# Clemapfel/kmer_index

Measured on NVIDIA B200. Metric: search_queries_per_s, higher is better.
Workload: dtype u32

## Files before the change

kmer_index_b200/csrc/build_kernels.cu:

```cuda
#include "radix.cuh"
#include "launch.h"

namespace kb {

__global__ void __launch_bounds__(256) pack_text_kernel(const uint8_t *__restrict__ ranks, uint64_t n, uint32_t bits,
                                                        uint32_t sigma, uint64_t n_words, uint64_t *__restrict__ words,
                                                        uint32_t *__restrict__ error_flag) {
    const uint64_t w = (uint64_t)blockIdx.x * blockDim.x + threadIdx.x;
    if (w >= n_words) return;
    const uint32_t spw = 64 / bits;
    const uint64_t s0 = w * spw;
    uint64_t word = 0;
    bool bad = false;
    if (s0 + spw <= n && ((uintptr_t)(ranks + s0) & 7) == 0) {
        const uint64_t *src = reinterpret_cast<const uint64_t *>(ranks + s0);
        for (uint32_t j = 0; j < spw; j += 8) {
            const uint64_t v = src[j >> 3];
#pragma unroll
            for (uint32_t b = 0; b < 8; ++b) {
                const uint32_t r = (uint32_t)(v >> (8 * b)) & 0xFF;
                bad |= r >= sigma;
                word |= (uint64_t)r << (64 - bits * (j + b + 1));
            }
        }
// ... 475 lines not shown
    const int tid = threadIdx.x;
    const uint64_t tile_begin = (uint64_t)blockIdx.x * kTile;
    const uint64_t tile_end = min(tile_begin + kTile, n_kmers + 1);
    const uint32_t nb = (uint32_t)(tile_end - tile_begin);
    const bool edge = tile_begin == 0 || tile_end == n_kmers + 1;

    const uint64_t i0 = tile_begin + (uint64_t)tid * ITEMS;
    const KeyT k_base = tile_begin ? keys[tile_begin - 1] : (KeyT)0;
    KeyT k[ITEMS + 1];
    k[0] = (i0 >= 1 && i0 - 1 < n_kmers) ? keys[i0 - 1] : (KeyT)0;
    if (i0 + ITEMS <= n_kmers) {
        constexpr int kPerVec = 16 / (int)sizeof(KeyT);
        const uint4 *p = reinterpret_cast<const uint4 *>(keys + i0);
#pragma unroll
        for (int v = 0; v < ITEMS / kPerVec; ++v) {
            const uint4 q = p[v];
            if (sizeof(KeyT) == 4) {
                k[1 + 4 * v] = (KeyT)q.x;
                k[2 + 4 * v] = (KeyT)q.y;
                k[3 + 4 * v] = (KeyT)q.z;
                k[4 + 4 * v] = (KeyT)q.w;
            } else {
                k[1 + 2 * v] = (KeyT)(((uint64_t)q.y << 32) | q.x);
                k[2 + 2 * v] = (KeyT)(((uint64_t)q.w << 32) | q.z);
            }
        }
    } else {
#pragma unroll
        for (int j = 0; j < ITEMS; ++j) k[j + 1] = (i0 + j < n_kmers) ? keys[i0 + j] : (KeyT)0;
    }
#pragma unroll
    for (int t = 0; t < kSlab / (kDirThreads * 4); ++t)
        *reinterpret_cast<uint4 *>(slab + (t * kDirThreads + tid) * 4) = make_uint4(0, 0, 0, 0);

    const uint32_t b0 = (uint32_t)tid * ITEMS;
    if (!edge) {
        const uint32_t slot_base = (uint32_t)(k_base >> shift);
        uint32_t rel[ITEMS + 1];
#pragma unroll
        for (int j = 0; j <= ITEMS; ++j) rel[j] = (uint32_t)(k[j] >> shift) - slot_base;
        uint32_t head[ITEMS];
#pragma unroll
        for (int j = 0; j < ITEMS; ++j) head[j] = rel[j + 1] > rel[j] ? rel[j] : 0xFFFFFFFFu;
        if (tid == kDirThreads - 1) s_end = rel[ITEMS];
        __syncthreads();
        directory_rounds<uint32_t, ITEMS>(slab, warp_last, head, (uint32_t)i0, (uint32_t)s_end,
                                          dir + ((uint64_t)slot_base + 1));
    } else {
        const uint64_t base = tile_begin ? (uint64_t)(k_base >> shift) + 1 : 0;
        uint64_t head[ITEMS];
#pragma unroll
        for (int j = 0; j < ITEMS; ++j) {
            const uint64_t i = i0 + j;
            head[j] = ~0ull;
            if (b0 + j < nb) {
                const uint64_t lo = (i == 0) ? 0 : (uint64_t)(k[j] >> shift) + 1;
                const uint64_t hi = (i == n_kmers) ? dir_entries : (uint64_t)(k[j + 1] >> shift) + 1;
                if (hi > lo) head[j] = lo - base;
                if (b0 + j == nb - 1) s_end = hi - base;
            }
        }
        __syncthreads();
        directory_rounds<uint64_t, ITEMS>(slab, warp_last, head, (uint32_t)i0, s_end, dir + base);
    }
}

template <typename KeyT, int ITEMS>
static void launch_directory_fill_t(const KeyT *d_keys, uint64_t n_kmers, uint32_t shift, uint64_t dir_entries, uint32_t *d_dir,
                                    cudaStream_t stream) {
    const uint64_t tile = (uint64_t)kDirThreads * ITEMS;
    const uint64_t blocks = (n_kmers + 1 + tile - 1) / tile;
    cudaFuncSetAttribute(directory_fill_kernel<KeyT, ITEMS>, cudaFuncAttributePreferredSharedMemoryCarveout, 100);
    directory_fill_kernel<KeyT, ITEMS><<<(unsigned)blocks, kDirThreads, 0, stream>>>(d_keys, n_kmers, shift, dir_entries, d_dir);
}

void launch_directory_fill(const void *d_keys, uint32_t key_bytes, uint64_t n_kmers, uint32_t shift, uint64_t dir_entries,
                           uint32_t *d_dir, cudaStream_t stream) {
    if (key_bytes == 8)
        launch_directory_fill_t<uint64_t, 8>((const uint64_t *)d_keys, n_kmers, shift, dir_entries, d_dir, stream);
    else
        launch_directory_fill_t<uint32_t, 8>((const uint32_t *)d_keys, n_kmers, shift, dir_entries, d_dir, stream);
}

template <typename Source, int BITS, bool BYTE>
static void launch_scatter_bits(const Source &src, uint64_t n, uint32_t shift, uint32_t mask, const uint32_t *d_tile_base,
                                typename Source::key_type *d_out_keys, uint32_t *d_out_vals, cudaStream_t stream) {
    using Smem = ScatterSmem<typename Source::key_type, (Source::kAtomicItems != 0)>;
    const uint32_t n_tiles = (uint32_t)((n + kSortTile - 1) / kSortTile);
    cudaFuncSetAttribute(radix_scatter_kernel<Source, BITS, BYTE>, cudaFuncAttributeMaxDynamicSharedMemorySize, (int)sizeof(Smem));
    radix_scatter_kernel<Source, BITS, BYTE>
        <<<n_tiles, kSortThreads, sizeof(Smem), stream>>>(src, n, shift, mask, d_tile_base, d_out_keys, d_out_vals);
}

template <typename Source>
static void launch_scatter(const Source &src, uint64_t n, uint32_t shift, uint32_t mask, const uint32_t *d_tile_base,
                           typename Source::key_type *d_out_keys, uint32_t *d_out_vals, cudaStream_t stream) {
    const int bits = __builtin_popcount(mask);
    if (bits <= 5)
        launch_scatter_bits<Source, 5, false>(src, n, shift, mask, d_tile_base, d_out_keys, d_out_vals, stream);
    else if (bits == 6)
        launch_scatter_bits<Source, 6, false>(src, n, shift, mask, d_tile_base, d_out_keys, d_out_vals, stream);
    else if (bits == 7)
        launch_scatter_bits<Source, 7, false>(src, n, shift, mask, d_tile_base, d_out_keys, d_out_vals, stream);
    else if (sizeof(typename Source::key_type) == 4 && (shift & 7) == 0) {
        if constexpr (sizeof(typename Source::key_type) == 4)
            launch_scatter_bits<Source, 8, true>(src, n, shift, mask, d_tile_base, d_out_keys, d_out_vals, stream);
    } else
        launch_scatter_bits<Source, 8, false>(src, n, shift, mask, d_tile_base, d_out_keys, d_out_vals, stream);
}

void launch_column_scan(uint32_t *d_tile_hist, uint32_t n_tiles, uint32_t *d_chunk_sums, cudaStream_t stream) {
    const uint32_t n_chunks = (n_tiles + kScanChunk - 1) / kScanChunk;
    column_sum_kernel<<<n_chunks, kRadix, 0, stream>>>(d_tile_hist, n_tiles, d_chunk_sums);
    column_base_kernel<<<1, kRadix * kBaseSlices, 0, stream>>>(d_chunk_sums, n_chunks);
    column_apply_kernel<<<n_chunks, kRadix, 0, stream>>>(d_tile_hist, n_tiles, d_chunk_sums);
}

void launch_hist_text(const PackedText &text, uint32_t k, uint64_t n_kmers, uint32_t shift, uint32_t mask,
                      uint32_t *d_tile_hist, cudaStream_t stream) {
    const uint32_t n_tiles = (uint32_t)((n_kmers + kSortTile - 1) / kSortTile);
    if (k * text.bits > 64) {
        radix_hist_kernel<<<n_tiles, kSortThreads, 0, stream>>>(WideTextSource{text, k}, n_kmers, shift, mask, d_tile_hist);
        return;
    }
    radix_hist_text_kernel<<<n_tiles, kSortThreads, 0, stream>>>(text, k, n_kmers, shift, mask, d_tile_hist);
}

void launch_hist_pairs(const void *d_keys, uint32_t key_bytes, uint64_t n, uint32_t shift, uint32_t mask,
                       uint32_t *d_tile_hist, cudaStream_t stream) {
    const uint32_t n_tiles = (uint32_t)((n + kSortTile - 1) / kSortTile);
    if (key_bytes == 8) {
        PairSource<uint64_t> src{(const uint64_t *)d_keys, nullptr};
        radix_hist_kernel<<<n_tiles, kSortThreads, 0, stream>>>(src, n, shift, mask, d_tile_hist);
    } else {
        radix_hist_keys32_kernel<<<n_tiles, kSortThreads, 0, stream>>>((const uint32_t *)d_keys, n, shift, mask, d_tile_hist);
    }
}

void launch_scatter_text(const PackedText &text, uint32_t k, uint32_t key_bytes, uint64_t n_kmers, uint32_t shift,
                         uint32_t mask, const uint32_t *d_tile_base, void *d_out_keys, uint32_t *d_out_vals,
                         cudaStream_t stream) {
    if (k * text.bits > 64)
        launch_scatter(WideTextSource{text, k}, n_kmers, shift, mask, d_tile_base, (uint64_t *)d_out_keys, d_out_vals, stream);
    else if (key_bytes == 8)
        launch_scatter(TextSource<uint64_t>{text, k}, n_kmers, shift, mask, d_tile_base, (uint64_t *)d_out_keys, d_out_vals, stream);
    else
        launch_scatter(TextSource<uint32_t>{text, k}, n_kmers, shift, mask, d_tile_base, (uint32_t *)d_out_keys, d_out_vals, stream);
}

void launch_scatter_pairs(const void *d_keys, const uint32_t *d_vals, uint32_t key_bytes, uint64_t n, uint32_t shift,
                          uint32_t mask, const uint32_t *d_tile_base, void *d_out_keys, uint32_t *d_out_vals,
                          cudaStream_t stream) {
    if (key_bytes == 8)
        launch_scatter(PairSource<uint64_t>{(const uint64_t *)d_keys, d_vals}, n, shift, mask, d_tile_base,
                       (uint64_t *)d_out_keys, d_out_vals, stream);
    else
        launch_scatter(PairSource<uint32_t>{(const uint32_t *)d_keys, d_vals}, n, shift, mask, d_tile_base,
                       (uint32_t *)d_out_keys, d_out_vals, stream);
}

uint32_t sort_tile_size() { return kSortTile; }
uint32_t scan_chunk_tiles() { return kScanChunk; }

}
```

kmer_index_b200/csrc/capi.cu:

```cuda
#include <algorithm>
#include <atomic>
#include <condition_variable>
#include <chrono>
#include <cmath>
#include <cstdio>
#include <cstdlib>
#include <cstring>
#include <mutex>
#include <unordered_map>
#include <new>
#include <string>
#include <system_error>
#include <thread>
#include <vector>

#include "host_pack.h"
#include "launch.h"
#include "radix.cuh"

namespace {

thread_local std::string g_last_error;

int fail(int code, const std::string &msg) {
// ... 340 lines not shown
    return p;
}

void pinned_put(void *p, size_t cap) {
    if (!p) return;
    {
        std::lock_guard<std::mutex> lock(g_pinned_mu);
        if (g_pinned_cache.size() < 32) {
            g_pinned_cache.emplace_back(p, cap);
            return;
        }
    }
    cudaFreeHost(p);
}

struct SchemeHost {
    std::vector<uint32_t> ks;
    std::vector<uint32_t> sum_off;
    std::vector<uint8_t> sum_elem, use_multi;
};

void build_scheme(SchemeHost *ix) {
    const uint32_t R = kb::kQuerySizeRange;
    std::vector<uint32_t> all_ks(ix->ks);
    std::sort(all_ks.begin(), all_ks.end(), [](uint32_t a, uint32_t b) { return a > b; });
    std::vector<uint32_t> high;
    for (uint32_t k : all_ks)
        if (k >= 9) high.push_back(k);
    std::vector<uint32_t> len(R, 0), last(R, 0), prev(R, 0);
    ix->use_multi.assign(R, 0);
    for (uint32_t k : high)
        if (k < R) {
            len[k] = 1;
            last[k] = k;
            ix->use_multi[k] = 1;
        }
    for (uint32_t q = all_ks.front() + 1; q < R; ++q)
        for (uint32_t k : high)
            if (len[q - k] != 0) {
                len[q] = len[q - k] + 1;
                last[q] = k;
                prev[q] = q - k;
                ix->use_multi[q] = 1;
                break;
            }
    for (uint32_t q = 0; q < R; ++q) {
        if (len[q] != 0) continue;
        uint32_t best = all_ks.front();
        if (q < all_ks.front()) {
            for (uint32_t k : all_ks)
                if (q <= k && k - q < best - q) best = k;
        } else {
            auto waste = [q](uint32_t k) { return ((q + k - 1) / k) * k - q; };
            for (uint32_t k : all_ks)
                if (waste(k) < waste(best)) best = k;
        }
        len[q] = 1;
        last[q] = best;
    }
    auto elem_of = [ix](uint32_t k) {
        for (size_t i = 0; i < ix->ks.size(); ++i)
            if (ix->ks[i] == k) return (uint8_t)i;
        return (uint8_t)0;
    };
    ix->sum_off.assign(R + 2, 0);
    uint64_t total = 0;
    for (uint32_t q = 0; q < R; ++q) {
        ix->sum_off[q] = (uint32_t)total;
        total += len[q];
    }
    ix->sum_off[R] = (uint32_t)total;
    ix->sum_off[R + 1] = (uint32_t)total;
    ix->sum_elem.assign(total, 0);
    for (uint32_t q = 0; q < R; ++q) {
        uint64_t o = (uint64_t)ix->sum_off[q] + len[q];
        uint32_t c = q;
        for (uint32_t j = 0; j < len[q]; ++j) {
            ix->sum_elem[--o] = elem_of(last[c]);
            c = prev[c];
        }
    }
}

int sort_element_tiled(kmer_b200_index *ix, uint32_t k, HostElement &he, uint32_t digit_bits, KeyRange part, uint64_t *n_sorted) {
    using namespace kb;
    cudaStream_t st = ix->stream;
    Profiler &pf = ix->prof;
    const uint64_t n_text_kmers = ix->n - k + 1;
    const uint32_t key_bytes = he.key_bytes;
    const bool partial = part.lo != 0 || part.hi != fast_pow(ix->sigma, (uint8_t)k);
    PackedText text{ix->d_text, ix->n, ix->bits, ix->sigma};
    uint64_t n_kmers = n_text_kmers;
    uint32_t sort_bits = he.key_bits;
    void *f_keys = nullptr;
    uint32_t *f_vals = nullptr;
    if (partial) {
        const uint32_t ft = filter_tiles(n_text_kmers);
        uint64_t *tile_counts = nullptr, *block_sums = nullptr;
        KB_TRY(dev_alloc(ix, &tile_counts, (uint64_t)ft + 1, false));
        KB_TRY(dev_alloc(ix, &block_sums, offsets_scan_blocks(ft) + 1, false));
        pf.begin(K_HIST_TEXT, (double)n_text_kmers * ix->bits / 8.0);
        launch_owned_count(text, k, n_text_kmers, part.lo, part.hi, tile_counts, st);
        pf.end();
        launch_offsets_scan(tile_counts, ft, block_sums, st);
        KB_CUDA(cudaMemcpyAsync(&ix->h_pinned[6], tile_counts + ft, sizeof(uint64_t), cudaMemcpyDeviceToHost, st));
        KB_CUDA(cudaStreamSynchronize(st));
        n_kmers = ix->h_pinned[6];
        KB_TRY(dev_alloc(ix, (uint8_t **)&f_keys, std::max<uint64_t>(n_kmers, 1) * key_bytes, true));
        KB_TRY(dev_alloc(ix, &f_vals, std::max<uint64_t>(n_kmers, 1), true));
        pf.begin(K_SCATTER_TEXT, (double)n_text_kmers * ix->bits / 8.0 + 8.0 * n_kmers);
        launch_owned_write(text, k, n_text_kmers, part.lo, part.hi, tile_counts, (uint32_t *)f_keys, f_vals, st);
        pf.end();
        dev_free(ix, tile_counts);
        dev_free(ix, block_sums);
        sort_bits = std::max<uint32_t>(1, bit_length(part.hi - part.lo - 1));
    }
    *n_sorted = n_kmers;
    he.sort_passes = (sort_bits + digit_bits - 1) / digit_bits;
    const uint32_t bits_per_pass = (sort_bits + he.sort_passes - 1) / he.sort_passes;
    const uint32_t mask = (1u << bits_per_pass) - 1;
    const uint32_t n_tiles = (uint32_t)((n_kmers + sort_tile_size() - 1) / sort_tile_size());
    const uint32_t n_chunks = (n_tiles + scan_chunk_tiles() - 1) / scan_chunk_tiles();
    const double text_bytes = (double)n_kmers * ix->bits / 8.0;
    const double hist_bytes = (double)n_tiles * kRadix * 4;
    void *keys[2] = {nullptr, nullptr};
    uint32_t *vals[2] = {nullptr, nullptr};
    uint32_t *tile_hist = nullptr, *chunk_sums = nullptr;
    auto alloc_keys = [&](void **p) { return dev_alloc(ix, (uint8_t **)p, std::max<uint64_t>(n_kmers, 1) * key_bytes, true); };
    KB_TRY(dev_alloc(ix, &tile_hist, (uint64_t)std::max(n_tiles, 1u) * kRadix, false));
    KB_TRY(dev_alloc(ix, &chunk_sums, (uint64_t)std::max(n_chunks, 1u) * kRadix, false));
    int cur = 0;
    uint32_t first_pair_pass = 1;
    if (partial) {
        keys[0] = f_keys;
        vals[0] = f_vals;
        first_pair_pass = 0;
    } else {
        KB_TRY(alloc_keys(&keys[0]));
        KB_TRY(dev_alloc(ix, &vals[0], n_kmers, true));
        pf.begin(K_HIST_TEXT, text_bytes + hist_bytes);
        launch_hist_text(text, k, n_kmers, 0, mask, tile_hist, st);
        pf.end();
        pf.begin(K_COLUMN_SCAN, 3 * hist_bytes, 3);
        launch_column_scan(tile_hist, n_tiles, chunk_sums, st);
        pf.end();
        pf.begin(K_SCATTER_TEXT, text_bytes + hist_bytes + (4.0 + key_bytes) * n_kmers);
        launch_scatter_text(text, k, key_bytes, n_kmers, 0, mask, tile_hist, keys[0], vals[0], st);
        pf.end();
    }
    for (uint32_t p = first_pair_pass; p < he.sort_passes && n_kmers > 0; ++p) {
        const int nxt = cur ^ 1;
        if (!keys[nxt]) {
            KB_TRY(alloc_keys(&keys[nxt]));
            KB_TRY(dev_alloc(ix, &vals[nxt], n_kmers, true));
        }
        const uint32_t shift = p * bits_per_pass;
        pf.begin(K_HIST_PAIRS, (double)key_bytes * n_kmers + hist_bytes);
        launch_hist_pairs(keys[cur], key_bytes, n_kmers, shift, mask, tile_hist, st);
        pf.end();
        pf.begin(K_COLUMN_SCAN, 3 * hist_bytes, 3);
        launch_column_scan(tile_hist, n_tiles, chunk_sums, st);
        pf.end();
        pf.begin(K_SCATTER_PAIRS, 2.0 * (4.0 + key_bytes) * n_kmers + hist_bytes);
        launch_scatter_pairs(keys[cur], vals[cur], key_bytes, n_kmers, shift, mask, tile_hist, keys[nxt], vals[nxt], st);
        pf.end();
        cur = nxt;
    }
    KB_CUDA(cudaGetLastError());
    if (keys[cur ^ 1]) {
        dev_free(ix, (uint8_t *)keys[cur ^ 1]);
        dev_free(ix, vals[cur ^ 1]);
        ix->device_bytes -= std::max<uint64_t>(n_kmers, 1) * (sizeof(uint32_t) + key_bytes);
    }
    dev_free(ix, tile_hist);
    dev_free(ix, chunk_sums);
    he.d_keys = keys[cur];
    he.d_pos = vals[cur];
    return 0;
}

int sort_element_onesweep(kmer_b200_index *ix, uint32_t k, HostElement &he, uint32_t digit_bits, uint64_t *n_sorted) {
    using namespace kb;
    cudaStream_t st = ix->stream;
    Profiler &pf = ix->prof;
    const uint64_t n_kmers = ix->n - k + 1;
    PackedText text{ix->d_text, ix->n, ix->bits, ix->sigma};
    const bool pow2 = ix->sigma == (1u << ix->bits);
    uint32_t passes = (he.key_bits + digit_bits - 1) / digit_bits;
    uint32_t w = (he.key_bits + passes - 1) / passes;
    if (pow2) {
        w = (w + ix->bits - 1) / ix->bits * ix->bits;
        if (w > (uint32_t)kRadixBitsMax) w = kRadixBitsMax / ix->bits * ix->bits;
        passes = (he.key_bits + w - 1) / w;
    }
    if (passes > 8) return fail(KMER_B200_ERR_UNSUPPORTED, "more than 8 digit passes");
    he.sort_passes = passes;
    const uint32_t mask = (1u << w) - 1;
    const uint32_t n_tiles = (uint32_t)((n_kmers + sort_tile_size() - 1) / sort_tile_size());
    const double text_bytes = (double)n_kmers * ix->bits / 8.0;
    const double status_bytes = 2.0 * (double)n_tiles * kRadix * 8;

    uint64_t *status = nullptr;
    uint32_t *scratch = nullptr;
    uint2 *pairs[2] = {nullptr, nullptr};
    uint32_t *keys = nullptr, *pos = nullptr;
    auto cleanup = [&](int code) {
        dev_free(ix, status);
        dev_free(ix, scratch);
        dev_free(ix, pairs[0]);
        dev_free(ix, pairs[1]);
        if (code != 0) {
            dev_free(ix, keys);
            dev_free(ix, pos);
        }
        return code;
    };
    if (dev_alloc(ix, &status, (uint64_t)n_tiles * kRadix, false) || dev_alloc(ix, &scratch, 4096 + 8, false))
        return cleanup(KMER_B200_ERR_OUT_OF_MEMORY);
    cudaMemsetAsync(status, 0, (uint64_t)n_tiles * kRadix * sizeof(uint64_t), st);
    cudaMemsetAsync(scratch + 4096, 0, 8 * sizeof(uint32_t), st);
    uint32_t *digit_base = scratch + 2048, *counters = scratch + 4096;

    pf.begin(K_HIST_TEXT, text_bytes, 2);
    launch_digit_histograms(text, k, n_kmers, passes, w, he.key_bits, pow2, scratch, digit_base, st);
    pf.end();

    int cur = -1;
    for (uint32_t p = 0; p < passes; ++p) {
        const bool last = p + 1 == passes;
        uint2 *out_pairs = nullptr;
        if (last) {
            if (cur >= 0 && pairs[cur ^ 1]) {
                dev_free(ix, pairs[cur ^ 1]);
                pairs[cur ^ 1] = nullptr;
            }
            if (dev_alloc(ix, &pos, n_kmers, true) || dev_alloc(ix, &keys, n_kmers, true)) return cleanup(KMER_B200_ERR_OUT_OF_MEMORY);
        } else {
            const int nxt = cur < 0 ? 0 : cur ^ 1;
            if (!pairs[nxt] && dev_alloc(ix, &pairs[nxt], n_kmers + 2, false)) return cleanup(KMER_B200_ERR_OUT_OF_MEMORY);
            out_pairs = pairs[nxt];
        }
        const double out_bytes = last ? 8.0 * n_kmers : 8.0 * n_kmers;
        if (p == 0) {
            pf.begin(K_SCATTER_TEXT, text_bytes + out_bytes + status_bytes);
            launch_onesweep_pass(&text, k, nullptr, n_kmers, 0, mask, 1, digit_base, status, counters, out_pairs, keys, pos, st);
        } else {
            pf.begin(K_SCATTER_PAIRS, 8.0 * n_kmers + out_bytes + status_bytes);
            launch_onesweep_pass(nullptr, k, pairs[cur], n_kmers, p * w, mask, p + 1, digit_base + p * kRadix, status, counters + p,
                                 out_pairs, keys, pos, st);
        }
        pf.end();
        if (!last) cur = cur < 0 ? 0 : cur ^ 1;
    }
    KB_CUDA(cudaGetLastError());
    he.d_keys = keys;
    he.d_pos = pos;
    *n_sorted = n_kmers;
    return cleanup(0);
}

int build_element(kmer_b200_index *ix, uint32_t k, HostElement &he, bool auxiliary = false) {
    using namespace kb;
    cudaStream_t st = ix->stream;
    Profiler &pf = ix->prof;
    const uint64_t n_kmers = ix->n - k + 1;
    const uint64_t key_space = fast_pow(ix->sigma, (uint8_t)k);
    he.key_bits = std::max<uint32_t>(1, bit_length(key_space - 1));
    uint32_t digit_bits = kRadixBitsMax;
    if (const char *env = std::getenv("KMER_B200_DIGIT_BITS")) {
        const int b = std::atoi(env);
        if (b >= 4 && b <= kRadixBitsMax) digit_bits = (uint32_t)b;
    }
    const uint32_t key_bytes = he.key_bits > 32 ? 8 : 4;
    he.key_bytes = key_bytes;
    const KeyRange part = key_range_of(ix->cfg, key_space);
    const bool partial = ix->cfg.key_parts > 1;
    if (partial && (key_bytes != 4 || k * ix->bits > 64))
        return fail(KMER_B200_ERR_UNSUPPORTED, "key-range parts need 32-bit hashes (sigma^k <= 2^32)");
    const uint64_t max_rel = (partial ? part.hi - part.lo : key_space) - 1;
    uint64_t n_part = n_kmers;
    const char *sorter = std::getenv("KMER_B200_SORT");
    if (!partial && key_bytes == 4 && k * ix->bits <= 64 && sorter && std::strcmp(sorter, "onesweep") == 0) {
        KB_TRY(sort_element_onesweep(ix, k, he, digit_bits, &n_part));
    } else {
        KB_TRY(sort_element_tiled(ix, k, he, digit_bits, part, &n_part));
    }

    uint32_t shift = 0;
    const uint32_t part_bits = std::max<uint32_t>(1, bit_length(max_rel));
    if (ix->cfg.directory_bits) {
        if (part_bits > ix->cfg.directory_bits) shift = part_bits - ix->cfg.directory_bits;
    } else {
        uint32_t want = bit_length(n_part) + 1;
        if (want < 16) want = 16;
        if (part_bits > want) {
            size_t free_b = 0, total_b = 0;
            cudaMemGetInfo(&free_b, &total_b);
            const bool affordable = (ix->sharded || partial) && max_rel < (1ull << 33) && max_rel * 4ull + (1ull << 30) < free_b / 3;
            if (!affordable) shift = part_bits - want;
        }
    }
    if (partial && shift != 0) return fail(KMER_B200_ERR_UNSUPPORTED, "key-range parts need a dense directory");
    if (part_bits > 32 + shift) shift = part_bits - 32;
    const uint64_t dir_entries = (max_rel >> shift) + 2;
    KB_TRY(dev_alloc(ix, &he.d_dir, dir_entries, true));
    pf.begin(K_DIRECTORY_FILL, (double)key_bytes * n_part + 4.0 * dir_entries);
    launch_directory_fill(he.d_keys, key_bytes, n_part, shift, dir_entries, he.d_dir, st);
    pf.end();
    KB_CUDA(cudaGetLastError());
    if (shift == 0) {
        dev_free(ix, (uint8_t *)he.d_keys);
        he.d_keys = nullptr;
        ix->device_bytes -= std::max<uint64_t>(n_part, 1) * key_bytes;
    }

    he.dev.k = k;
    he.dev.shift = shift;
    he.dev.n_kmers = n_part;
    he.dev.dir_entries = dir_entries;
    he.dev.key_space = key_space;
    he.dev.dir = he.d_dir;
    he.dev.keys = he.d_keys;
    he.dev.pos = he.d_pos;
    he.dev.key_bytes = key_bytes;
    he.dev.key_lo = partial ? part.lo : 0;
    he.dev.key_hi = partial ? part.hi : UINT64_MAX;
    he.dev.k_phys = k;
    he.dev.width = 1;
    he.bytes = n_part * (sizeof(uint32_t) + (he.d_keys ? key_bytes : 0)) + dir_entries * sizeof(uint32_t);
    if (!auxiliary)
        ix->max_avg_bucket = std::max(ix->max_avg_bucket, (double)n_kmers / (double)std::min<uint64_t>(key_space, n_kmers));
    return 0;
}

#define KB_CUDA_RET(expr)                                                                           \
    do {                                                                                            \
        cudaError_t _e = (expr);                                                                    \
        if (_e != cudaSuccess) {                                                                    \
            cudaGetLastError();                                                                     \
            return fail(_e == cudaErrorMemoryAllocation ? KMER_B200_ERR_OUT_OF_MEMORY : KMER_B200_ERR_CUDA, \
                        std::string(#expr) + ": " + cudaGetErrorString(_e));                        \
        }                                                                                           \
    } while (0)

int new_index(uint64_t n, uint32_t sigma, const uint32_t *ks, uint32_t n_ks, const kmer_b200_config *cfg_in,
              kmer_b200_index **out) {
    *out = nullptr;
    if (!ks) return fail(KMER_B200_ERR_INVALID_ARGUMENT, "ks is null");
    if (n_ks == 0 || n_ks > (uint32_t)kb::kMaxElements)
        return fail(KMER_B200_ERR_INVALID_ARGUMENT, "number of ks must be in [1, 32]");
    if (sigma < 2 || sigma > 256) return fail(KMER_B200_ERR_INVALID_ARGUMENT, "sigma must be in [2, 256]");
    const uint32_t bits = sigma <= 4 ? 2 : (sigma <= 16 ? 4 : 8);
    uint32_t k_max = 0;
    for (uint32_t i = 0; i < n_ks; ++i) {
        const uint32_t k = ks[i];
        if (k == 0 || !((double)k < 64.0 / std::log2((double)sigma)))
            return fail(KMER_B200_ERR_INVALID_ARGUMENT, "k must satisfy 0 < k < 64 / log2(sigma) (kmer_index.hpp:42)");
        for (uint32_t j = 0; j < i; ++j)
            if (ks[j] == k) return fail(KMER_B200_ERR_INVALID_ARGUMENT, "duplicate k");
        k_max = std::max(k_max, k);
    }
    if (n < k_max) return fail(KMER_B200_ERR_INVALID_ARGUMENT, "text shorter than the largest k");
    kmer_b200_config cfg;
    if (cfg_in)
        cfg = *cfg_in;
    else
        kmer_b200_config_default(&cfg);
    const uint64_t n_total = cfg.n_total ? cfg.n_total : n;
    if (cfg.shard_begin + n > n_total) return fail(KMER_B200_ERR_INVALID_ARGUMENT, "shard exceeds n_total");
    if (n_total >= 0xFFFFFFFFull) return fail(KMER_B200_ERR_INVALID_ARGUMENT, "text too large for 32-bit positions");
    const bool sharded = cfg.n_total != 0 && (cfg.shard_begin != 0 || n != n_total);
    const bool reaches_end = cfg.shard_begin + n == n_total;
    if (cfg.halo >= n && cfg.halo) return fail(KMER_B200_ERR_INVALID_ARGUMENT, "halo must be smaller than the slice");
    if (sharded && !reaches_end && cfg.halo + 1 < k_max)
        return fail(KMER_B200_ERR_INVALID_ARGUMENT, "interior shards need halo >= max k - 1");

    if (cfg.key_parts > 1 && cfg.key_part >= cfg.key_parts) return fail(KMER_B200_ERR_INVALID_ARGUMENT, "key_part must be < key_parts");
    if (cfg.key_parts > 1 && sharded) return fail(KMER_B200_ERR_INVALID_ARGUMENT, "key-range parts index the whole text: no position-range shard");
    if ((cfg.reserved & KMER_B200_FLAG_SHARED_POSITIONS) && n_ks > 1) {
        if (sharded || cfg.key_parts > 1 || cfg.n_devices > 1)
            return fail(KMER_B200_ERR_UNSUPPORTED, "a shared-positions index is unsharded and lives on one device");
        cfg.reserved |= KMER_B200_FLAG_NO_AUX;
    } else {
        cfg.reserved &= ~(uint32_t)KMER_B200_FLAG_SHARED_POSITIONS;
    }
    int device = cfg.device;
    if (device < 0) {
        cudaError_t e = cudaGetDevice(&device);
        if (e != cudaSuccess) {
            cudaGetLastError();
            return fail(KMER_B200_ERR_CUDA, std::string("cudaGetDevice: ") + cudaGetErrorString(e));
        }
    }
// ... 3008 lines not shown
```

kmer_index_b200/csrc/launch.h:

```cpp
#pragma once

#include "common.cuh"

namespace kb {

void launch_pack_text(const uint8_t *d_ranks, uint64_t n, uint32_t bits, uint32_t sigma, uint64_t n_words_total,
                      uint64_t *d_words, uint32_t *d_error_flag, cudaStream_t stream);
void launch_hist_text(const PackedText &text, uint32_t k, uint64_t n_kmers, uint32_t shift, uint32_t mask,
                      uint32_t *d_tile_hist, cudaStream_t stream);
void launch_hist_pairs(const void *d_keys, uint32_t key_bytes, uint64_t n, uint32_t shift, uint32_t mask,
                       uint32_t *d_tile_hist, cudaStream_t stream);
void launch_column_scan(uint32_t *d_tile_hist, uint32_t n_tiles, uint32_t *d_chunk_sums, cudaStream_t stream);
void launch_scatter_text(const PackedText &text, uint32_t k, uint32_t key_bytes, uint64_t n_kmers, uint32_t shift,
                         uint32_t mask, const uint32_t *d_tile_base, void *d_out_keys, uint32_t *d_out_vals,
                         cudaStream_t stream);
void launch_scatter_pairs(const void *d_keys, const uint32_t *d_vals, uint32_t key_bytes, uint64_t n, uint32_t shift,
                          uint32_t mask, const uint32_t *d_tile_base, void *d_out_keys, uint32_t *d_out_vals,
                          cudaStream_t stream);
void launch_directory_fill(const void *d_keys, uint32_t key_bytes, uint64_t n_kmers, uint32_t shift, uint64_t dir_entries,
                           uint32_t *d_dir, cudaStream_t stream);
uint32_t sort_tile_size();
uint32_t scan_chunk_tiles();
void launch_digit_histograms(const PackedText &text, uint32_t k, uint64_t n_kmers, uint32_t n_passes, uint32_t w_bits,
                             uint32_t key_bits, bool from_cmers, uint32_t *d_hist_scratch, uint32_t *d_digit_base,
                             cudaStream_t stream);
void launch_onesweep_pass(const PackedText *text, uint32_t k, const uint2 *d_in_pairs, uint64_t n, uint32_t shift, uint32_t mask,
                          uint32_t tag, const uint32_t *d_digit_base, uint64_t *d_status, uint32_t *d_tile_counter,
                          uint2 *d_out_pairs, uint32_t *d_out_keys, uint32_t *d_out_vals, cudaStream_t stream);
uint32_t device_sm_count();
uint32_t filter_tiles(uint64_t n_kmers);
void launch_owned_count(const PackedText &text, uint32_t k, uint64_t n_kmers, uint64_t lo, uint64_t hi, uint64_t *d_tile_counts,
                        cudaStream_t stream);
void launch_owned_write(const PackedText &text, uint32_t k, uint64_t n_kmers, uint64_t lo, uint64_t hi, const uint64_t *d_tile_offsets,
                        uint32_t *d_out_keys, uint32_t *d_out_vals, cudaStream_t stream);
void launch_digit_histograms_pairs(const uint2 *d_pairs, uint64_t n, uint32_t n_passes, uint32_t w_bits, uint32_t *d_hist_scratch,
                                   uint32_t *d_digit_base, cudaStream_t stream);

enum SearchPass : int {
    kPassCount = 0,
    kPassWrite = 1,
    kPassPresence = 2,
    kPassCountAccount = 3,
    kPassCountDeferred = 4,
    kPassCountDeferredAccount = 5
};

struct SearchArgs {
    const DeviceIndex *index;
    const uint8_t *q_ranks;
    const uint64_t *q_offsets;
    const uint64_t *q_packed;
    const uint16_t *q_lens16;
    uint32_t q_stride;
    uint64_t n_queries;
    uint32_t mode;
    uint32_t group;
    uint32_t bits;
    uint32_t single_k;
    uint32_t lean_ok;
    struct {
        uint32_t n;
        uint32_t first[kMaxPosParts + 1];
        const uint32_t *ptr[kMaxPosParts];
    } parts0;
    uint32_t views;
    uint32_t *heavy;
    uint32_t *hits;
    uint32_t q_words;
    uint32_t max_len;
    const uint64_t *present_global;
    const uint32_t *present_global4;
    uint32_t *present4;
    uint64_t *counts;
    uint8_t *status;
    uint8_t *unsorted;
    uint32_t *positions;
    uint8_t *defer;
    uint64_t *present;
    unsigned long long *gather_count;
    uint32_t *error_flag;
    uint32_t approx;
    uint32_t max_mismatches;
};

constexpr uint32_t kHeavyCandidates = 2048;

void launch_search(const SearchArgs &args, SearchPass pass, cudaStream_t stream);
constexpr uint32_t kMaxMismatches = 8;
void launch_search_approx(const SearchArgs &args, SearchPass pass, cudaStream_t stream);
enum ApproxMode : int { kApproxAll = 0, kApproxListed = 1, kApproxBest = 2 };
struct ApproxHitArgs {
    uint8_t *budget;
    uint8_t *best_dist;
    uint32_t *best_pos;
    uint32_t strata;
};
void launch_search_approx_hits(const SearchArgs &args, const ApproxHitArgs &h, ApproxMode mode, SearchPass pass,
                               cudaStream_t stream);
void launch_approx_single(const SearchArgs &args, const ApproxHitArgs &h, uint8_t *d_distances, cudaStream_t stream);
void launch_approx_distances(const SearchArgs &args, const ApproxHitArgs &h, uint8_t *d_distances, cudaStream_t stream);
uint32_t search_q_words(uint32_t group, uint32_t bits, uint64_t max_len);
void launch_finalize_deferred(uint64_t *d_counts, uint8_t *d_status, const uint8_t *d_defer, const uint32_t *d_present4_global,
                              uint64_t n_queries, cudaStream_t stream);
// ... 58 lines not shown
```

Measured before the change: 16.30 billion.

## Fuse final radix pass with directory construction in a bucket-finish kernel

When the key fits 32 bits and the directory is dense, the LSD sort skips the lowest 8-bit digit. A new finish kernel instead sorts each high-digit bucket locally in shared memory and writes the directory entries at the same time, with a separate two-phase kernel for buckets that overflow a tile. This removes one full global radix pass and the separate directory-fill kernel at build time. The workload metric is search throughput, though, so this build-side change may not affect what is measured, and the finish path adds considerable complexity.

```diff
diff --git a/kmer_index_b200/csrc/build_kernels.cu b/kmer_index_b200/csrc/build_kernels.cu
--- a/kmer_index_b200/csrc/build_kernels.cu
+++ b/kmer_index_b200/csrc/build_kernels.cu
@@ -581,6 +581,279 @@
         launch_directory_fill_t<uint32_t, 8>((const uint32_t *)d_keys, n_kmers, shift, dir_entries, d_dir, stream);
 }
 
+constexpr int kFinThreads = 256;
+constexpr int kFinWarps = kFinThreads / 32;
+constexpr int kFinTile = 4096;
+constexpr int kFinStage = 6144;
+constexpr uint32_t kFinOpen = 0xFFFFFFFFu;
+constexpr int kHeavyBlocks = 32;
+constexpr uint32_t kFinBucketMax = 64;
+
+struct FinishSmem {
+    uint32_t val[kFinStage];
+    uint16_t out[kFinStage];
+    uint32_t cnt[kFinWarps][kRadix];
+    uint32_t beg[kFinWarps][kRadix];
+    uint32_t flags[kFinTile / 32];
+    uint16_t runs[kFinTile];
+    uint8_t dig[kFinStage];
+    uint32_t n_runs, end;
+};
+
+__device__ __forceinline__ void dir_fill_range(uint32_t *__restrict__ dir, uint64_t lo, uint64_t hi, uint32_t v) {
+    const int lane = threadIdx.x & 31;
+    for (uint64_t h = lo + lane; h < hi; h += 32) dir[h] = v;
+}
+
+__device__ __forceinline__ uint32_t dir_block_from_hist(uint32_t *counts, uint32_t *begin, uint32_t *__restrict__ dir,
+                                                        uint64_t B, uint64_t start, uint64_t dir_entries, uint32_t cursor0) {
+    const int lane = threadIdx.x & 31;
+    uint32_t c[8], sum = 0, most = 0;
+#pragma unroll
+    for (int j = 0; j < 8; ++j) {
+        c[j] = counts[lane * 8 + j];
+        sum += c[j];
+        most = max(most, c[j]);
+    }
+    uint32_t incl = sum;
+#pragma unroll
+    for (int o = 1; o < 32; o <<= 1) {
+        const uint32_t v = __shfl_up_sync(0xFFFFFFFFu, incl, o);
+        if (lane >= o) incl += v;
+    }
+    uint32_t e = incl - sum;
+    const uint64_t h0 = B * kRadix + lane * 8;
+    uint32_t d[8];
+#pragma unroll
+    for (int j = 0; j < 8; ++j) {
+        d[j] = (uint32_t)start + e;
+        counts[lane * 8 + j] = cursor0 + e;
+        begin[lane * 8 + j] = cursor0 + e;
+        e += c[j];
+    }
+    if (h0 + 8 <= dir_entries) {
+        uint4 *p = reinterpret_cast<uint4 *>(dir + h0);
+        p[0] = make_uint4(d[0], d[1], d[2], d[3]);
+        p[1] = make_uint4(d[4], d[5], d[6], d[7]);
+    } else {
+#pragma unroll
+        for (int j = 0; j < 8; ++j)
+            if (h0 + j < dir_entries) dir[h0 + j] = d[j];
+    }
+    __syncwarp();
+    return __reduce_max_sync(0xFFFFFFFFu, most);
+}
+
+__device__ __forceinline__ uint32_t rank_chunk(uint32_t *cursor, uint32_t d, bool valid) {
+    const int lane = threadIdx.x & 31;
+    const uint32_t peers = match_digit<8>(d, __ballot_sync(0xFFFFFFFFu, valid));
+    const uint32_t below = (uint32_t)__popc(peers & ((1u << lane) - 1));
+    const uint32_t base = valid ? cursor[d] : 0u;
+    __syncwarp();
+    if (valid && (peers >> lane) == 1u) cursor[d] = base + (uint32_t)__popc(peers);
+    __syncwarp();
+    return base + below;
+}
+
+__global__ void __launch_bounds__(kFinThreads) directory_finish_kernel(const uint32_t *__restrict__ keys,
+                                                                       uint32_t *__restrict__ vals_pos, uint64_t n,
+                                                                       uint64_t dir_entries, uint32_t *__restrict__ dir,
+                                                                       uint32_t *__restrict__ heavy) {
+    extern __shared__ __align__(16) unsigned char smem_raw[];
+    FinishSmem &sm = *reinterpret_cast<FinishSmem *>(smem_raw);
+    const int tid = threadIdx.x, lane = tid & 31, warp = tid >> 5;
+    const uint64_t t0 = (uint64_t)blockIdx.x * kFinTile;
+    const uint32_t tn = (uint32_t)min((uint64_t)kFinTile, n - t0);
+    if (tid == 0) {
+        sm.n_runs = 0;
+        sm.end = kFinOpen;
+    }
+    constexpr int kItems = kFinTile / kFinThreads;
+    uint32_t key[kItems], val[kItems], before[kItems];
+#pragma unroll
+    for (int r = 0; r < kItems; ++r) {
+        const uint32_t i = r * kFinThreads + tid;
+        key[r] = i < tn ? keys[t0 + i] : 0u;
+        val[r] = i < tn ? vals_pos[t0 + i] : 0u;
+        before[r] = (lane == 0 && i < tn && t0 + i > 0) ? keys[t0 + i - 1] : 0u;
+    }
+    __syncthreads();
+#pragma unroll
+    for (int r = 0; r < kItems; ++r) {
+        const uint32_t i = r * kFinThreads + tid;
+        const bool in = i < tn;
+        uint32_t prev = __shfl_up_sync(0xFFFFFFFFu, key[r], 1);
+        if (lane == 0) prev = before[r];
+        const bool start = in && (t0 + i == 0 || (key[r] >> 8) != (prev >> 8));
+        const uint32_t b = __ballot_sync(0xFFFFFFFFu, start);
+        if (lane == 0 && in) sm.flags[i >> 5] = b;
+        if (in) {
+            sm.dig[i] = (uint8_t)key[r];
+            sm.val[i] = val[r];
+        }
+        if (start) {
+            sm.runs[atomicAdd(&sm.n_runs, 1u)] = (uint16_t)i;
+        }
+    }
+    __syncthreads();
+    if (sm.n_runs == 0) return;
+    if (t0 + tn < n) {
+        const uint32_t hl = keys[t0 + tn - 1] >> 8;
+        uint32_t ra = tn;
+        for (;;) {
+            const uint32_t i = ra + tid;
+            bool stop = false;
+            if (i < kFinStage && t0 + i < n) {
+                const uint32_t key = keys[t0 + i];
+                const uint32_t v = vals_pos[t0 + i];
+                if ((key >> 8) == hl) {
+                    sm.dig[i] = (uint8_t)key;
+                    sm.val[i] = v;
+                } else {
+                    atomicMin(&sm.end, i);
+                    stop = true;
+                }
+            }
+            ra += kFinThreads;
+            if (__syncthreads_or(stop)) break;
+            if (t0 + ra >= n && n - t0 <= kFinStage) {
+                if (tid == 0) sm.end = (uint32_t)(n - t0);
+                break;
+            }
+            if (ra >= kFinStage) break;
+        }
+    } else if (tid == 0) {
+        sm.end = tn;
+    }
+    __syncthreads();
+    const uint32_t end_last = sm.end;
+
+    uint32_t *cursor = sm.cnt[warp];
+    for (uint32_t r = warp; r < sm.n_runs; r += kFinWarps) {
+        const uint32_t a = sm.runs[r];
+        const uint64_t ga = t0 + a;
+        const uint64_t B = keys[ga] >> 8;
+        const uint64_t gap_lo = ga ? ((uint64_t)(keys[ga - 1] >> 8) + 1) * kRadix : 0;
+        uint32_t b = end_last;
+        for (uint32_t w0 = (a + 1) >> 5; w0 * 32 < tn; w0 += 32) {
+            const uint32_t w = w0 + lane;
+            uint32_t bits = w * 32 < tn ? sm.flags[w] : 0u;
+            if (w == ((a + 1) >> 5)) bits &= 0xFFFFFFFFu << ((a + 1) & 31);
+            const uint32_t any = __ballot_sync(0xFFFFFFFFu, bits != 0);
+            if (any) {
+                const int src = __ffs(any) - 1;
+                b = (w0 + src) * 32 + __ffs(__shfl_sync(0xFFFFFFFFu, bits, src)) - 1;
+                break;
+            }
+        }
+        dir_fill_range(dir, gap_lo, min(B * kRadix, dir_entries), (uint32_t)ga);
+        if (b == kFinOpen) {
+            if (lane == 0) heavy[1 + 2 * atomicAdd(heavy, 1u)] = (uint32_t)ga;
+            continue;
+        }
+#pragma unroll
+        for (int j = 0; j < kRadix / 32; ++j) cursor[j * 32 + lane] = 0;
+        __syncwarp();
+        for (uint32_t i = a + lane; i < b; i += 32) atomicAdd(&cursor[sm.dig[i]], 1u);
+        __syncwarp();
+        const uint32_t *begin = sm.beg[warp];
+        const bool ordered = dir_block_from_hist(cursor, sm.beg[warp], dir, B, ga, dir_entries, a) > kFinBucketMax;
+        if (ordered) {
+            for (uint32_t c = a; c < b; c += 32) {
+                const uint32_t i = c + lane;
+                const bool valid = i < b;
+                const uint32_t dst = rank_chunk(cursor, valid ? sm.dig[i] : 0u, valid);
+                if (valid) sm.out[dst] = (uint16_t)i;
+            }
+        } else {
+            for (uint32_t i = a + lane; i < b; i += 32) sm.out[atomicAdd(&cursor[sm.dig[i]], 1u)] = (uint16_t)i;
+            __syncwarp();
+        }
+        for (uint32_t s = a + lane; s < b; s += 32) {
+            const uint32_t i = sm.out[s];
+            uint32_t dst = s;
+            if (!ordered) {
+                const uint32_t d = sm.dig[i];
+                const uint32_t lo = begin[d], hi = cursor[d];
+                dst = lo;
+                for (uint32_t t = lo; t < hi; ++t) dst += sm.out[t] < i;
+            }
+            vals_pos[t0 + dst] = sm.val[i];
+        }
+        __syncwarp();
+        if (t0 + b == n) dir_fill_range(dir, (B + 1) * kRadix, dir_entries, (uint32_t)n);
+    }
+}
+
+template <bool PLACE>
+__global__ void __launch_bounds__(kFinThreads) directory_finish_heavy_kernel(uint32_t *__restrict__ keys,
+                                                                             uint32_t *__restrict__ vals_pos, uint64_t n,
+                                                                             uint64_t dir_entries, uint32_t *__restrict__ dir,
+                                                                             uint32_t *__restrict__ heavy, PackedText text,
+                                                                             uint32_t k, uint32_t key_lo) {
+    __shared__ uint32_t cnt[kFinWarps][kRadix];
+    const int lane = threadIdx.x & 31, warp = threadIdx.x >> 5;
+    uint32_t *cursor = cnt[warp];
+    const uint32_t n_heavy = heavy[0];
+    for (uint32_t h = blockIdx.x * kFinWarps + warp; h < n_heavy; h += gridDim.x * kFinWarps) {
+        const uint64_t a = heavy[1 + 2 * h];
+        const uint64_t B = keys[a] >> 8;
+        if (!PLACE) {
+#pragma unroll
+            for (int j = 0; j < kRadix / 32; ++j) cursor[j * 32 + lane] = 0;
+            __syncwarp();
+            uint64_t b = a;
+            for (;;) {
+                const uint64_t i = b + lane;
+                const uint32_t key = i < n ? keys[i] : 0u;
+                const bool member = i < n && (key >> 8) == B;
+                if (member) atomicAdd(&cursor[key & 0xFF], 1u);
+                const uint32_t m = __ballot_sync(0xFFFFFFFFu, member);
+                b += __popc(m);
+                if (m != 0xFFFFFFFFu) break;
+            }
+            __syncwarp();
+            if (lane == 0) heavy[2 + 2 * h] = (uint32_t)b;
+            dir_block_from_hist(cursor, cursor, dir, B, a, dir_entries, (uint32_t)a);
+            if (b == n) dir_fill_range(dir, (B + 1) * kRadix, dir_entries, (uint32_t)n);
+        } else {
+            const uint64_t b = heavy[2 + 2 * h];
+#pragma unroll
+            for (int j = 0; j < kRadix / 32; ++j) {
+                const uint64_t e = B * kRadix + j * 32 + lane;
+                cursor[j * 32 + lane] = e < dir_entries ? dir[e] : 0u;
+            }
+            __syncwarp();
+            for (uint64_t c = a; c < b; c += 32) {
+                const uint64_t i = c + lane;
+                const bool valid = i < b;
+                const uint32_t p = valid ? vals_pos[i] : 0u;
+                const uint32_t d = valid ? (uint32_t)(key_from_window(window64(text.words, p, text.bits), k, text.bits, text.sigma) - key_lo) & 0xFFu : 0u;
+                const uint32_t dst = rank_chunk(cursor, d, valid);
+                if (valid) keys[dst] = p;
+            }
+            __syncwarp();
+            for (uint64_t i = a + lane; i < b; i += 32) vals_pos[i] = keys[i];
+        }
+    }
+}
+
+uint64_t directory_finish_heavy_words(uint64_t n_kmers) { return 1 + 2 * ((n_kmers + kFinTile - 1) / kFinTile); }
+
+void launch_directory_finish(uint32_t *d_keys, uint32_t *d_vals_pos, uint64_t n_kmers, uint64_t dir_entries, uint32_t *d_dir,
+                             uint32_t *d_heavy, const PackedText &text, uint32_t k, uint32_t key_lo, cudaStream_t stream) {
+    cudaMemsetAsync(d_heavy, 0, sizeof(uint32_t), stream);
+    const uint64_t blocks = (n_kmers + kFinTile - 1) / kFinTile;
+    cudaFuncSetAttribute(directory_finish_kernel, cudaFuncAttributeMaxDynamicSharedMemorySize, (int)sizeof(FinishSmem));
+    cudaFuncSetAttribute(directory_finish_kernel, cudaFuncAttributePreferredSharedMemoryCarveout, 100);
+    directory_finish_kernel<<<(unsigned)blocks, kFinThreads, sizeof(FinishSmem), stream>>>(d_keys, d_vals_pos, n_kmers,
+                                                                                             dir_entries, d_dir, d_heavy);
+    directory_finish_heavy_kernel<false><<<kHeavyBlocks, kFinThreads, 0, stream>>>(d_keys, d_vals_pos, n_kmers, dir_entries,
+                                                                                  d_dir, d_heavy, text, k, key_lo);
+    directory_finish_heavy_kernel<true><<<kHeavyBlocks, kFinThreads, 0, stream>>>(d_keys, d_vals_pos, n_kmers, dir_entries,
+                                                                                 d_dir, d_heavy, text, k, key_lo);
+}
+
 template <typename Source, int BITS, bool BYTE>
 static void launch_scatter_bits(const Source &src, uint64_t n, uint32_t shift, uint32_t mask, const uint32_t *d_tile_base,
                                 typename Source::key_type *d_out_keys, uint32_t *d_out_vals, cudaStream_t stream) {
diff --git a/kmer_index_b200/csrc/capi.cu b/kmer_index_b200/csrc/capi.cu
--- a/kmer_index_b200/csrc/capi.cu
+++ b/kmer_index_b200/csrc/capi.cu
@@ -446,7 +446,28 @@
     }
 }
 
-int sort_element_tiled(kmer_b200_index *ix, uint32_t k, HostElement &he, uint32_t digit_bits, KeyRange part, uint64_t *n_sorted) {
+uint32_t directory_shift(kmer_b200_index *ix, uint64_t n_part, uint64_t max_rel, bool partial, uint64_t pending_bytes) {
+    uint32_t shift = 0;
+    const uint32_t part_bits = std::max<uint32_t>(1, bit_length(max_rel));
+    if (ix->cfg.directory_bits) {
+        if (part_bits > ix->cfg.directory_bits) shift = part_bits - ix->cfg.directory_bits;
+    } else {
+        uint32_t want = bit_length(n_part) + 1;
+        if (want < 16) want = 16;
+        if (part_bits > want) {
+            size_t free_b = 0, total_b = 0;
+            cudaMemGetInfo(&free_b, &total_b);
+            free_b -= std::min<uint64_t>(free_b, pending_bytes);
+            const bool affordable = (ix->sharded || partial) && max_rel < (1ull << 33) && max_rel * 4ull + (1ull << 30) < free_b / 3;
+            if (!affordable) shift = part_bits - want;
+        }
+    }
+    if (part_bits > 32 + shift) shift = part_bits - 32;
+    return shift;
+}
+
+int sort_element_tiled(kmer_b200_index *ix, uint32_t k, HostElement &he, uint32_t digit_bits, KeyRange part, uint64_t max_rel,
+                       uint64_t *n_sorted, uint64_t *dir_entries_out) {
     using namespace kb;
     cudaStream_t st = ix->stream;
     Profiler &pf = ix->prof;
@@ -480,8 +501,13 @@
         sort_bits = std::max<uint32_t>(1, bit_length(part.hi - part.lo - 1));
     }
     *n_sorted = n_kmers;
-    he.sort_passes = (sort_bits + digit_bits - 1) / digit_bits;
-    const uint32_t bits_per_pass = (sort_bits + he.sort_passes - 1) / he.sort_passes;
+    const bool finish_shape = key_bytes == 4 && k * ix->bits <= 64 && sort_bits > kRadixBitsMax;
+    const bool finish = finish_shape && directory_shift(ix, n_kmers, max_rel, partial,
+                                                        partial ? 0 : std::max<uint64_t>(n_kmers, 1) * (4 + key_bytes)) == 0;
+    const uint32_t low_bits = finish ? kRadixBitsMax : 0;
+    const uint32_t lsd_passes = (sort_bits - low_bits + digit_bits - 1) / digit_bits;
+    he.sort_passes = lsd_passes + (finish ? 1 : 0);
+    const uint32_t bits_per_pass = (sort_bits - low_bits + lsd_passes - 1) / lsd_passes;
     const uint32_t mask = (1u << bits_per_pass) - 1;
     const uint32_t n_tiles = (uint32_t)((n_kmers + sort_tile_size() - 1) / sort_tile_size());
     const uint32_t n_chunks = (n_tiles + scan_chunk_tiles() - 1) / scan_chunk_tiles();
@@ -503,22 +529,22 @@
         KB_TRY(alloc_keys(&keys[0]));
         KB_TRY(dev_alloc(ix, &vals[0], n_kmers, true));
         pf.begin(K_HIST_TEXT, text_bytes + hist_bytes);
-        launch_hist_text(text, k, n_kmers, 0, mask, tile_hist, st);
+        launch_hist_text(text, k, n_kmers, low_bits, mask, tile_hist, st);
         pf.end();
         pf.begin(K_COLUMN_SCAN, 3 * hist_bytes, 3);
         launch_column_scan(tile_hist, n_tiles, chunk_sums, st);
         pf.end();
         pf.begin(K_SCATTER_TEXT, text_bytes + hist_bytes + (4.0 + key_bytes) * n_kmers);
-        launch_scatter_text(text, k, key_bytes, n_kmers, 0, mask, tile_hist, keys[0], vals[0], st);
+        launch_scatter_text(text, k, key_bytes, n_kmers, low_bits, mask, tile_hist, keys[0], vals[0], st);
         pf.end();
     }
-    for (uint32_t p = first_pair_pass; p < he.sort_passes && n_kmers > 0; ++p) {
+    for (uint32_t p = first_pair_pass; p < lsd_passes && n_kmers > 0; ++p) {
         const int nxt = cur ^ 1;
         if (!keys[nxt]) {
             KB_TRY(alloc_keys(&keys[nxt]));
             KB_TRY(dev_alloc(ix, &vals[nxt], n_kmers, true));
         }
-        const uint32_t shift = p * bits_per_pass;
+        const uint32_t shift = low_bits + p * bits_per_pass;
         pf.begin(K_HIST_PAIRS, (double)key_bytes * n_kmers + hist_bytes);
         launch_hist_pairs(keys[cur], key_bytes, n_kmers, shift, mask, tile_hist, st);
         pf.end();
@@ -540,6 +566,25 @@
     dev_free(ix, chunk_sums);
     he.d_keys = keys[cur];
     he.d_pos = vals[cur];
+    *dir_entries_out = 0;
+    if (!finish) return 0;
+    const uint64_t dir_entries = max_rel + 2;
+    uint32_t *heavy = nullptr;
+    KB_TRY(dev_alloc(ix, &he.d_dir, dir_entries, true));
+    KB_TRY(dev_alloc(ix, &heavy, directory_finish_heavy_words(n_kmers), false));
+    pf.begin(K_DIRECTORY_FILL, 12.0 * n_kmers + 4.0 * dir_entries);
+    if (n_kmers)
+        launch_directory_finish((uint32_t *)keys[cur], vals[cur], n_kmers, dir_entries, he.d_dir, heavy, text, k,
+                                (uint32_t)part.lo, st);
+    else
+        KB_CUDA(cudaMemsetAsync(he.d_dir, 0, dir_entries * sizeof(uint32_t), st));
+    pf.end();
+    KB_CUDA(cudaGetLastError());
+    dev_free(ix, heavy);
+    dev_free(ix, (uint8_t *)keys[cur]);
+    ix->device_bytes -= std::max<uint64_t>(n_kmers, 1) * key_bytes;
+    he.d_keys = nullptr;
+    *dir_entries_out = dir_entries;
     return 0;
 }
 
@@ -643,36 +688,26 @@
         return fail(KMER_B200_ERR_UNSUPPORTED, "key-range parts need 32-bit hashes (sigma^k <= 2^32)");
     const uint64_t max_rel = (partial ? part.hi - part.lo : key_space) - 1;
     uint64_t n_part = n_kmers;
+    uint64_t dir_entries = 0;
     const char *sorter = std::getenv("KMER_B200_SORT");
     if (!partial && key_bytes == 4 && k * ix->bits <= 64 && sorter && std::strcmp(sorter, "onesweep") == 0) {
         KB_TRY(sort_element_onesweep(ix, k, he, digit_bits, &n_part));
     } else {
-        KB_TRY(sort_element_tiled(ix, k, he, digit_bits, part, &n_part));
+        KB_TRY(sort_element_tiled(ix, k, he, digit_bits, part, max_rel, &n_part, &dir_entries));
     }
 
     uint32_t shift = 0;
-    const uint32_t part_bits = std::max<uint32_t>(1, bit_length(max_rel));
-    if (ix->cfg.directory_bits) {
-        if (part_bits > ix->cfg.directory_bits) shift = part_bits - ix->cfg.directory_bits;
-    } else {
-        uint32_t want = bit_length(n_part) + 1;
-        if (want < 16) want = 16;
-        if (part_bits > want) {
-            size_t free_b = 0, total_b = 0;
-            cudaMemGetInfo(&free_b, &total_b);
-            const bool affordable = (ix->sharded || partial) && max_rel < (1ull << 33) && max_rel * 4ull + (1ull << 30) < free_b / 3;
-            if (!affordable) shift = part_bits - want;
-        }
-    }
-    if (partial && shift != 0) return fail(KMER_B200_ERR_UNSUPPORTED, "key-range parts need a dense directory");
-    if (part_bits > 32 + shift) shift = part_bits - 32;
-    const uint64_t dir_entries = (max_rel >> shift) + 2;
-    KB_TRY(dev_alloc(ix, &he.d_dir, dir_entries, true));
-    pf.begin(K_DIRECTORY_FILL, (double)key_bytes * n_part + 4.0 * dir_entries);
-    launch_directory_fill(he.d_keys, key_bytes, n_part, shift, dir_entries, he.d_dir, st);
-    pf.end();
-    KB_CUDA(cudaGetLastError());
-    if (shift == 0) {
+    if (!dir_entries) {
+        shift = directory_shift(ix, n_part, max_rel, partial, 0);
+        if (partial && shift != 0) return fail(KMER_B200_ERR_UNSUPPORTED, "key-range parts need a dense directory");
+        dir_entries = (max_rel >> shift) + 2;
+        KB_TRY(dev_alloc(ix, &he.d_dir, dir_entries, true));
+        pf.begin(K_DIRECTORY_FILL, (double)key_bytes * n_part + 4.0 * dir_entries);
+        launch_directory_fill(he.d_keys, key_bytes, n_part, shift, dir_entries, he.d_dir, st);
+        pf.end();
+        KB_CUDA(cudaGetLastError());
+    }
+    if (shift == 0 && he.d_keys) {
         dev_free(ix, (uint8_t *)he.d_keys);
         he.d_keys = nullptr;
         ix->device_bytes -= std::max<uint64_t>(n_part, 1) * key_bytes;
diff --git a/kmer_index_b200/csrc/launch.h b/kmer_index_b200/csrc/launch.h
--- a/kmer_index_b200/csrc/launch.h
+++ b/kmer_index_b200/csrc/launch.h
@@ -19,6 +19,9 @@
                           cudaStream_t stream);
 void launch_directory_fill(const void *d_keys, uint32_t key_bytes, uint64_t n_kmers, uint32_t shift, uint64_t dir_entries,
                            uint32_t *d_dir, cudaStream_t stream);
+void launch_directory_finish(uint32_t *d_keys, uint32_t *d_vals_pos, uint64_t n_kmers, uint64_t dir_entries, uint32_t *d_dir,
+                             uint32_t *d_heavy, const PackedText &text, uint32_t k, uint32_t key_lo, cudaStream_t stream);
+uint64_t directory_finish_heavy_words(uint64_t n_kmers);
 uint32_t sort_tile_size();
 uint32_t scan_chunk_tiles();
 void launch_digit_histograms(const PackedText &text, uint32_t k, uint64_t n_kmers, uint32_t n_passes, uint32_t w_bits,
```

Result: no change. 16.34 billion (median of 6 runs) (+0.3%).
